# pranshu-raj-211/dmdqn

Measured on NVIDIA B200. Metric: agent-updates/sec, higher is better.
Workload: dtype f32

## Files before the change

dmdqn_b200/csrc/api.cu:

```cuda
#include <stdarg.h>
#include <string.h>
#include "common.cuh"

namespace dmdqn {

static thread_local char g_error[512] = "";

void set_error(const char* fmt, ...) {
    va_list ap;
    va_start(ap, fmt);
    vsnprintf(g_error, sizeof(g_error), fmt, ap);
    va_end(ap);
}

int validate_dims(const dmdqn_dims* d) {
    DMDQN_CHECK_ARG(d != nullptr, "dims is NULL");
    DMDQN_CHECK_ARG(d->n_agents >= 1, "n_agents=%d must be >= 1", d->n_agents);
    DMDQN_CHECK_ARG(d->n_nets == d->n_agents || d->n_nets == 1,
                    "n_nets=%d must be n_agents (independent) or 1 (shared)", d->n_nets);
    DMDQN_CHECK_ARG(d->obs_dim >= 1 && d->obs_stride >= d->obs_dim && d->obs_stride % 16 == 0 &&
                        d->obs_stride <= 128,
                    "obs_dim=%d obs_stride=%d: stride must be a multiple of 16 in [obs_dim, 128]",
                    d->obs_dim, d->obs_stride);
    DMDQN_CHECK_ARG(d->hidden == 64 || d->hidden == 128 || d->hidden == 256 || d->hidden == 512,
// ... 132 lines not shown

static int check_learn_args(const dmdqn_dims* dims, const dmdqn_hparams* hp, const dmdqn_replay* replay,
                            const dmdqn_nets* nets, const void* draws) {
    DMDQN_CHECK_ARG(hp && replay && nets && draws, "NULL argument");
    if (int rc = check_n_step(hp)) return rc;
    DMDQN_CHECK_ARG(replay->obs && replay->next_obs && replay->act && replay->rew && replay->done &&
                        replay->n_written, "NULL replay pointer");
    DMDQN_CHECK_ARG(nets->theta && nets->theta_tgt && nets->adam_m && nets->adam_v && nets->learn_step,
                    "NULL network pointer");
    DMDQN_CHECK_ARG(hp->sample_mode >= 0 && hp->sample_mode <= DMDQN_SAMPLE_PRIORITIZED, "sample_mode=%d", hp->sample_mode);
    if (hp->sample_mode == DMDQN_SAMPLE_PRIORITIZED) {
        DMDQN_CHECK_ARG(replay->priority && replay->priority_max,
                        "sample_mode=prioritized needs the replay's priority and priority_max arrays (NULL priority pointer)");
        DMDQN_CHECK_ARG(!(dims->n_nets == 1 && dims->n_agents > 1),
                        "sample_mode=prioritized serves independent networks only (n_nets=%d, n_agents=%d share parameters)",
                        dims->n_nets, dims->n_agents);
    }
    DMDQN_CHECK_ARG(hp->loss == DMDQN_LOSS_MSE || hp->loss == DMDQN_LOSS_HUBER, "loss=%d", hp->loss);
    DMDQN_CHECK_ARG(hp->precision >= DMDQN_PRECISION_FP32 && hp->precision <= DMDQN_PRECISION_TF32X3, "precision=%d",
                    hp->precision);
    return DMDQN_OK;
}

static int run_learn(const dmdqn_dims* dims, const dmdqn_hparams* hp, const dmdqn_replay* replay, const dmdqn_nets* nets,
                     const void* draws, const uint8_t* learn_mask, float* metrics_out, void* workspace,
                     size_t workspace_bytes, int32_t stages, float* grads, int32_t global_batch, void* stream) {
    Workspace w;
    int rc = check_workspace(dims, workspace, workspace_bytes, &w);
    if (rc) return rc;
    rc = check_learn_args(dims, hp, replay, nets, draws);
    if (rc) return rc;
    if (grads) DMDQN_CHECK_ARG(global_batch >= dims->batch, "global_batch=%d < batch=%d", global_batch, dims->batch);
    if (stages & DMDQN_STAGE_SAMPLE) {
        rc = launch_sample(*dims, *hp, *replay, *nets, draws, learn_mask, 1, (char*)workspace, w, (cudaStream_t)stream);
        if (rc) return rc;
    }
    return launch_learn(*dims, *hp, *replay, *nets, metrics_out, (char*)workspace, w, stages, grads, global_batch,
                        (cudaStream_t)stream);
}

int dmdqn_sample(const dmdqn_dims* dims, const dmdqn_hparams* hp, const dmdqn_replay* replay,
                 const dmdqn_nets* nets, const void* draws, const uint8_t* learn_mask, int32_t advance_step,
                 void* workspace, size_t workspace_bytes, void* stream) {
    Workspace w;
    int rc = check_workspace(dims, workspace, workspace_bytes, &w);
    if (rc) return rc;
    rc = check_learn_args(dims, hp, replay, nets, draws);
    if (rc) return rc;
    return launch_sample(*dims, *hp, *replay, *nets, draws, learn_mask, advance_step, (char*)workspace, w,
                         (cudaStream_t)stream);
}

int dmdqn_gather(const dmdqn_dims* dims, const dmdqn_replay* replay, const void* workspace,
                 size_t workspace_bytes, float* states, int32_t* actions, float* rewards, float* next_states,
                 float* dones, int32_t* active_out, void* stream) {
    Workspace w;
    int rc = check_workspace(dims, const_cast<void*>(workspace), workspace_bytes, &w);
    if (rc) return rc;
    DMDQN_CHECK_ARG(replay && replay->obs && replay->next_obs, "gather: NULL replay pointer");
    DMDQN_CHECK_ARG(states && actions && rewards && next_states && dones, "gather: NULL output");
    return launch_gather(*dims, *replay, (const char*)workspace, w, states, actions, rewards, next_states, dones,
                         active_out, (cudaStream_t)stream);
}

int dmdqn_learn_stages(const dmdqn_dims* dims, const dmdqn_hparams* hp, const dmdqn_replay* replay,
                       const dmdqn_nets* nets, const void* draws, const uint8_t* learn_mask, float* metrics_out,
                       void* workspace, size_t workspace_bytes, int32_t stages, void* stream) {
    return run_learn(dims, hp, replay, nets, draws, learn_mask, metrics_out, workspace, workspace_bytes, stages, nullptr, 0,
                     stream);
}

int dmdqn_learn(const dmdqn_dims* dims, const dmdqn_hparams* hp, const dmdqn_replay* replay,
                const dmdqn_nets* nets, const void* draws, const uint8_t* learn_mask, float* metrics_out,
                void* workspace, size_t workspace_bytes, void* stream) {
    return run_learn(dims, hp, replay, nets, draws, learn_mask, metrics_out, workspace, workspace_bytes, kAllStages, nullptr,
                     0, stream);
}

int dmdqn_step_host(const dmdqn_dims* dims, const dmdqn_hparams* hp, const dmdqn_replay* replay,
                    const dmdqn_nets* nets, const dmdqn_step_block* blk, const void* host_block, void* device_block,
                    float* metrics_dev, float* metrics_host, void* workspace, size_t workspace_bytes, void* stream) {
    int rc = validate_dims(dims);
// ... 140 lines not shown
```

dmdqn_b200/csrc/common.cuh:

```cuda
#pragma once
#include <cuda_runtime.h>
#include <stdint.h>
#include <stdio.h>
#include "../../include/dmdqn_b200.h"

namespace dmdqn {

void set_error(const char* fmt, ...);

#define DMDQN_CHECK_ARG(cond, ...)                                  \
    do {                                                            \
        if (!(cond)) {                                              \
            ::dmdqn::set_error(__VA_ARGS__);                        \
            return DMDQN_ERR_ARG;                                   \
        }                                                           \
    } while (0)

#define DMDQN_CUDA(expr)                                                              \
    do {                                                                              \
        cudaError_t _e = (expr);                                                      \
        if (_e != cudaSuccess) {                                                      \
            ::dmdqn::set_error("%s failed: %s", #expr, cudaGetErrorString(_e));       \
            return DMDQN_ERR_CUDA;                                                    \
        }                                                                             \
// ... 46 lines not shown
    int tiles;
};
inline int tile_bm(int h) { return h >= 512 ? 32 : 64; }
inline Workspace make_workspace(const dmdqn_dims& d) {
    Workspace w;
    size_t off = 0;
    auto take = [&](size_t bytes) { size_t o = off; off += (bytes + 255) / 256 * 256; return o; };
    const size_t nb = (size_t)d.n_nets * d.batch;
    w.tiles = row_tiles(d.batch, tile_bm(d.hidden));
    const size_t nt = (size_t)d.n_nets * w.tiles;
    w.rows = take(nb * 4);
    w.r_hat = take(nb * 4);
    w.act_b = take(nb * 4);
    w.done_b = take(nb * 4);
    w.active = take((size_t)d.n_nets * 4);
    w.y = take(nb * 4);
    w.q_all = take(nb * 16);
    w.q_next = take(nb * 16);
    w.tq_all = take(nb * 16);
    w.h1 = take(nb * d.hidden * 4);
    w.tc_error = take(4);
    w.adam_sc = take((size_t)d.n_nets * 16);
    w.mask2 = take(nb * (size_t)(d.hidden / 32) * 4);
    w.ga = take(nb * 8);
    w.w3_copy = take((size_t)d.n_nets * d.hidden * 16);
    w.dh1 = take(nb * d.hidden * 4);
    w.dh2 = take(nb * d.hidden * 4);
    w.part_loss = take(nt * 8 * 4);
    w.part_b3 = take(nt * 4 * 4);
    w.part_w3 = take(nt * d.hidden * 4 * 4);
    w.part_b2 = take(nt * d.hidden * 4);
    w.part_b1 = take(nt * d.hidden * 4);
    w.is_w = take(nb * 4);
    w.sync = take((4 + (size_t)d.n_nets + nt) * 4);
    w.nrows = take(nb * 4);
    w.disc_b = take(nb * 4);
    w.total = off;
    return w;
}

int validate_dims(const dmdqn_dims* d);

constexpr int kAllStages = DMDQN_STAGE_SAMPLE | DMDQN_STAGE_TARGET | DMDQN_STAGE_ONLINE | DMDQN_STAGE_WGRAD;

struct LearnArgs {
    dmdqn_dims d;
    Layout L;
    dmdqn_replay rp;
    dmdqn_nets nets;
    int loss, double_dqn;
    int loss_batch;
    float one_m_b1, one_m_b2, tau;
    int ws_tiles;
    int tc_tiles;
    const int32_t *rows, *nrows, *act_b, *active;
    const float *r_hat, *disc_b;
    const float4* adam_sc;
    float *y, *q_all, *q_next, *tq_all, *h1, *dh1, *dh2;
    float *part_loss, *part_b3, *part_w3, *part_b2, *part_b1;
    uint32_t* mask2;
    float2* ga;
    float* w3_copy;
    int* error;
    float* metrics;
    float* grads;
    int chain;
    int *sched, *k4a_done, *k3_done;
    int per;
    const float* is_w;
    double per_alpha, per_eps;
};
LearnArgs make_learn_args(const dmdqn_dims& d, const dmdqn_hparams& hp, const dmdqn_replay& rp, const dmdqn_nets& nets,
                          char* ws, const Workspace& w, float* metrics, float* grads, int loss_batch);

__device__ __forceinline__ void per_store_priority(const LearnArgs& A, int row, float delta) {
    const float p = (float)pow(fabs((double)delta) + A.per_eps, A.per_alpha);
    if (!isfinite(p)) return;
    A.rp.priority[row] = p;
    atomicMax(reinterpret_cast<int*>(A.rp.priority_max) + row / A.d.capacity, __float_as_int(p));
}

struct AdamStep {
    float alpha, eps, one_m_b1, one_m_b2, tau;
    int sync;
};
__device__ __forceinline__ AdamStep adam_step(const LearnArgs& A, int g) {
    const float4 sc = __ldg(A.adam_sc + g);
    return {sc.x, sc.y, A.one_m_b1, A.one_m_b2, A.tau, __float_as_int(sc.z)};
}

template <typename Load>
__device__ __forceinline__ void finish_metrics(const LearnArgs& A, int g, int tiles, Load ld) {
    double ls = 0, qs = 0, qq = 0, hist[4] = {0, 0, 0, 0};
#pragma unroll 1
    for (int r = 0; r < tiles; ++r) {
        const float* pl = A.part_loss + ((size_t)g * tiles + r) * 8;
        ls += ld(pl); qs += ld(pl + 1); qq += ld(pl + 2);
        for (int a = 0; a < 4; ++a) hist[a] += ld(pl + 3 + a);
    }
    const double cnt = (double)A.d.batch * A.d.n_actions, mean = qs / cnt, var = fmax(qq / cnt - mean * mean, 0.0);
    float* m = A.metrics + g * DMDQN_METRICS_STRIDE;
    m[0] = (float)(ls / A.loss_batch);
    m[1] = (float)mean;
    m[2] = (float)sqrt(var);
    for (int a = 0; a < 4; ++a) m[3 + a] = (float)hist[a];
    m[7] = 1.f;
}

constexpr int kMaxDevices = 64;
int device_sm_count(int* n_sm);
int opt_in_dynamic_smem(const void* kernel, size_t bytes, size_t (&cache)[kMaxDevices]);

int launch_featurize(int32_t n, const int32_t* halting, const int32_t* phase, const double* next_switch,
                     const double* phase_dur, double sim_time, const uint8_t* signal_valid,
                     const int32_t* nbr_idx, const int32_t* phase_lut, const double* snapshot,
                     double lw, double gw, double* own_out, float* obs_out, int32_t obs_out_stride,
                     double* reward_out, double* global_out, int64_t* scratch, cudaStream_t s);
int launch_featurize_alt(int32_t n, const int32_t* halting, const int32_t* phase, const double* next_switch,
                         const uint8_t* signal_valid, double sim_time, const int32_t* nbr_idx, const double* prev_own,
                         double* own_out, float* obs_out, int32_t obs_out_stride, double* reward_out, cudaStream_t s);
int launch_act(const dmdqn_dims& d, const dmdqn_nets& nets, const float* obs, int32_t stride,
               const double* eps, const uint32_t* w1, const uint32_t* w2, int32_t* actions, float* q_out,
               cudaStream_t s);
int launch_push(const dmdqn_dims& d, const dmdqn_replay& rp, const float* obs, const int32_t* act,
                const double* rew, const float* next_obs, const uint8_t* done, int32_t in_stride,
                const uint8_t* mask, cudaStream_t s);
int launch_sample(const dmdqn_dims& d, const dmdqn_hparams& hp, const dmdqn_replay& rp, const dmdqn_nets& nets,
                  const void* draws, const uint8_t* learn_mask, int advance, char* ws, const Workspace& w,
                  cudaStream_t s);
int launch_gather(const dmdqn_dims& d, const dmdqn_replay& rp, const char* ws, const Workspace& w,
                  float* states, int32_t* actions, float* rewards, float* next_states, float* dones,
                  int32_t* active_out, cudaStream_t s);
int launch_learn(const dmdqn_dims& d, const dmdqn_hparams& hp, const dmdqn_replay& rp, const dmdqn_nets& nets,
                 float* metrics, char* ws, const Workspace& w, int stages, float* grads, int loss_batch, cudaStream_t s);
bool tc_supported(const dmdqn_dims& d);
int launch_learn_tc(const LearnArgs& A, int precision, int stages, cudaStream_t s);
int launch_adam_apply(const dmdqn_dims& d, const dmdqn_hparams& hp, const dmdqn_nets& nets, const float* grads, char* ws,
                      const Workspace& w, cudaStream_t s);
int launch_sync_target(const dmdqn_dims& d, const dmdqn_nets& nets, const uint8_t* mask, double tau,
                       cudaStream_t s);
int launch_peer_adam(const dmdqn_dims& d, const dmdqn_hparams& hp, const dmdqn_nets& nets, const dmdqn_peers& peers,
                     const float* my_loss_src, float* loss_out, char* ws, const Workspace& w, cudaStream_t s);

}
```

dmdqn_b200/csrc/learn_tc.cu:

```cuda
#include <cuda.h>
#include <string.h>
#include "common.cuh"

namespace dmdqn {

namespace {

constexpr int H = 256;
constexpr int BM = 128;
constexpr int EW = 16;
constexpr int NT = EW * 32;
constexpr int W_MMA = EW, W_TMA = EW + 1, W_CONV = EW + 2;
constexpr int CONV_WARPS = 6, CONV_GROUP_WARPS = 2;
constexpr int NT_F = (EW + 8) * 32;
constexpr int REGS_EPI = 104, REGS_AUX = 32;
constexpr int KC = 16;
constexpr uint32_t ATOM = BM * 128;
constexpr unsigned long long WAIT_LIMIT_NS = 2000000000ull;

__device__ __forceinline__ uint32_t smem_u32(const void* p) { return (uint32_t)__cvta_generic_to_shared(p); }

__device__ __forceinline__ uint64_t make_desc(uint32_t saddr, uint32_t lbo_bytes, uint32_t sbo_bytes, uint32_t layout) {
    return (uint64_t)((saddr >> 4) & 0x3FFF) | (uint64_t)((lbo_bytes >> 4) & 0x3FFF) << 16 |
           (uint64_t)((sbo_bytes >> 4) & 0x3FFF) << 32 | (uint64_t)1 << 46 | (uint64_t)layout << 61;
// ... 491 lines not shown
__global__ void __launch_bounds__(NT_F, 1) tc_target_kernel(const LearnArgs A, const __grid_constant__ CUtensorMap tm_w1,
                                                            const __grid_constant__ CUtensorMap tm_w2,
                                                            const __grid_constant__ CUtensorMap tm_w1t,
                                                            const __grid_constant__ CUtensorMap tm_w2t) {
    extern __shared__ uint8_t smem_raw[];
    const uint32_t sbase = (smem_u32(smem_raw) + 1023u) & ~1023u;
    const int B = A.d.batch, Dp = A.d.obs_stride;
    const int n_items = 2 * A.d.n_nets * A.tc_tiles;
    const int warp = threadIdx.x >> 5;
    KT_BEGIN;
    const uint32_t tmem = tc_prologue(sbase);
    if (A.chain) {
        asm volatile("griddepcontrol.wait;" ::: "memory");
        pdl_launch_dependents();
    }
    Ring ring;
    bool ok = true;
    if (warp >= EW) {
        regs_dec<REGS_AUX>();
      if (warp == W_MMA) {
        if ((threadIdx.x & 31) == 0) {
            int prev = -1;
            for (int q = k3_next(A, blockIdx.x, n_items); q < n_items; q = k3_next(A, q + gridDim.x, n_items)) {
                ok = mma_gemm<PASSES, false>(sbase, tmem, sbase + Fwd::R, sbase + Fwd::XLO, 0, Dp, ring, ok);
                if (prev >= 0) flag_release_add(A.k3_done + (size_t)((prev >> 1) / A.tc_tiles) * A.ws_tiles + (prev >> 1) % A.tc_tiles);
                prev = q;
                ok = mma_gemm<PASSES, false>(sbase, tmem, sbase + Fwd::R, 0, tmem + 256u, H, ring, ok);
            }
            if (!ok) atomicExch(A.error, 13);
        }
        __syncwarp();
      } else if (warp == W_TMA) {
        if ((threadIdx.x & 31) == 0) {
            for (int q = k3_next(A, blockIdx.x, n_items); q < n_items;) {
                const int g = (q >> 1) / A.tc_tiles;
                const float* P = ((q & 1) ? A.nets.theta_tgt : A.nets.theta) + (size_t)g * A.L.stride;
                const int qn = k3_next(A, q + gridDim.x, n_items);
                const float* Pn = qn < n_items ? ((qn & 1) ? A.nets.theta_tgt : A.nets.theta) + (size_t)((qn >> 1) / A.tc_tiles) * A.L.stride + A.L.w1 : nullptr;
                ok = tma_fwd(sbase, (q & 1) ? &tm_w1t : &tm_w1, g, P + A.L.w1, Dp, ring, ok, P + A.L.w2);
                ok = tma_fwd(sbase, (q & 1) ? &tm_w2t : &tm_w2, g, P + A.L.w2, H, ring, ok, Pn);
                q = qn;
            }
            if (!ok) atomicExch(A.error, 23);
        }
        __syncwarp();
      } else if (warp < W_CONV + CONV_WARPS) {
        const int tc = threadIdx.x - W_CONV * 32, cg = (warp - W_CONV) / CONV_GROUP_WARPS, t = tc % (CONV_GROUP_WARPS * 32);
        for (int q = k3_next(A, blockIdx.x, n_items); q < n_items; q = k3_next(A, q + gridDim.x, n_items)) {
            ok = conv_ring<PASSES>(sbase, cg, t, ring, ok, Dp / 8);
            ok = conv_ring<PASSES>(sbase, cg, t, ring, ok, H / 8);
        }
        if (!ok && tc == 0) atomicExch(A.error, 33);
      }
    } else {
        regs_inc<REGS_EPI>();
        const Epi e;
        XGather<PASSES> xg;
        int q = k3_next(A, blockIdx.x, n_items);
        if (q < n_items) {
            const int g = (q >> 1) / A.tc_tiles, rt = (q >> 1) % A.tc_tiles;
            xg.begin(A.rp.next_obs, A.nrows + (size_t)g * B, rt * BM, B, Dp, ((q & 1) ? A.nets.theta_tgt : A.nets.theta) + (size_t)g * A.L.stride, A.L);
        }
        int q_last = -1;
        while (q < n_items) {
            const int item = q >> 1, pass = q & 1;
            const int g = item / A.tc_tiles, rt = item % A.tc_tiles, r0 = rt * BM;
// ... 388 lines not shown
    q = __shfl_sync(0xffffffffu, q, 0);
    if (q < 0) ok = __shfl_sync(0xffffffffu, (int)ok, 0) != 0;
    return q;
}
__device__ __forceinline__ float ldcg_f(const float* p) {
    float v;
    asm volatile("ld.global.cg.f32 %0, [%1];" : "=f"(v) : "l"(p));
    return v;
}

template <int PASSES>
__global__ void __launch_bounds__(Wg::NTW, 1) tc_wgrad_kernel(const LearnArgs A, const __grid_constant__ CUtensorMap tmap_h1,
                                                              const __grid_constant__ CUtensorMap tmap_dh1) {
    extern __shared__ uint8_t smem_raw[];
    const int B = A.d.batch, Dp = A.d.obs_stride, G = A.d.n_nets;
    const int tid = threadIdx.x, warp = tid >> 5, lane = tid & 31;
    const uint32_t sbase = (smem_u32(smem_raw) + 1023u) & ~1023u;
    const uint32_t bars = sbase + Wg::BARS;
    const int n_items = 3 * G;
    const int nchunks = (B + KC - 1) / KC;

    if (tid == 0) {
        for (int s = 0; s < Wg::STAGES; ++s) {
            mbar_init(bars + Wg::FULL + 8 * s, 1);
            mbar_init(bars + Wg::CONV + 8 * s, Wg::CONV_WARPS);
            mbar_init(bars + Wg::EMPTY + 8 * s, 1);
        }
        for (int b = 0; b < 2; ++b) {
            mbar_init(bars + Wg::ACC_FULL + 8 * b, 1);
            mbar_init(bars + Wg::ACC_FREE + 8 * b, Wg::EPI_WARPS);
        }
        for (int b = 0; b < Wg::NQ; ++b) mbar_init(bars + Wg::QFULL + 8 * b, 1);
        asm volatile("fence.mbarrier_init.release.cluster;" ::: "memory");
    }
    if (warp == 0) {
        asm volatile("tcgen05.alloc.cta_group::1.sync.aligned.shared::cta.b32 [%0], %1;" ::"r"(bars + Wg::TMEM), "r"(512));
        asm volatile("tcgen05.relinquish_alloc_permit.cta_group::1.sync.aligned;" ::);
    }
    tc_fence_before();
    __syncthreads();
    tc_fence_after();
    uint32_t tmem;
    asm volatile("ld.shared.u32 %0, [%1];" : "=r"(tmem) : "r"(bars + Wg::TMEM));
    bool ok = true;

    if (warp >= Wg::EPI_WARPS + Wg::CONV_WARPS) {
        regs_dec<Wg::REGS_AUX>();
        if (warp == Wg::EPI_WARPS + Wg::CONV_WARPS) {
            {
                uint32_t used = 0;
                int n = 0, nq = 0;
                for (;;) {
                    const int q = wg_pop(bars, nq, ok);
                    if (q < 0) break;
                    if (lane != 0) continue;
                    int g, t;
                    wg_item(q, G, g, t);
                    const bool is_w2 = t < 2;
                    const uint32_t acc_buf = (uint32_t)(n & 1);
                    const uint32_t d_tmem = tmem + acc_buf * 256u;
                    const uint32_t idesc = make_idesc(!is_w2, is_w2);
                    if (n >= 2 && ok)
                        ok = mbar_wait(bars + Wg::ACC_FREE + 8 * acc_buf, (uint32_t)((n >> 1) - 1) & 1u);
                    for (int c = 0; c < nchunks; ++c) {
                        const uint32_t s = used % Wg::STAGES, u = used / Wg::STAGES;
                        if (ok) ok = mbar_wait(bars + Wg::CONV + 8 * s, u & 1u);
                        tc_fence_after();
                        const uint32_t st = sbase + s * Wg::STG;
#pragma unroll
                        for (int ks = 0; ks < 2; ++ks) {
                            uint64_t a_hi, a_lo, b_hi, b_lo;
                            if (is_w2) {
                                a_hi = make_desc(st + ks * 32, 16, 512, 4);
                                a_lo = make_desc(st + Wg::A_BYTES + ks * 32, 16, 512, 4);
// ... 8 lines not shown
                            uint32_t acc = (c | ks) ? 1u : 0u;
                            if (PASSES == 3) {
                                mma_ss(d_tmem, a_lo, b_hi, idesc, acc);
                                mma_ss(d_tmem, a_hi, b_lo, idesc, 1u);
                                acc = 1u;
                            }
                            mma_ss(d_tmem, a_hi, b_hi, idesc, acc);
                        }
                        umma_commit(bars + Wg::EMPTY + 8 * s);
                        if (c == nchunks - 1) umma_commit(bars + Wg::ACC_FULL + 8 * acc_buf);
                        ++used;
                    }
                    ++n;
                }
                if (!ok && lane == 0) atomicExch(A.error, 15);
            }
            __syncwarp();
        } else if (warp == Wg::EPI_WARPS + Wg::CONV_WARPS + 1) {
            uint32_t used = 0;
            int nq = 0;
            int draws = 0;
            for (;;) {
                int q = (int)blockIdx.x + draws * (int)gridDim.x;
                ++draws;
                if (A.chain) {
                    if (lane == 0) q = atomicAdd(A.sched, 1);
                    q = __shfl_sync(0xffffffffu, q, 0);
                }
                if (q >= n_items || !ok) break;
                int g, t;
                wg_item(q, G, g, t);
                if (!A.active[g]) {
                    if (t == 2 && lane < DMDQN_METRICS_STRIDE && A.metrics) A.metrics[g * DMDQN_METRICS_STRIDE + lane] = 0.f;
                    continue;
                }
                if (A.chain) {
                    int fine = 1;
                    if (lane == 0) {
                        fine = flag_acquire_ge(A.k4a_done + g, A.tc_tiles) ? 1 : 0;
                        asm volatile("fence.proxy.async;" ::: "memory");
                    }
                    ok = __shfl_sync(0xffffffffu, fine, 0) != 0;
                    if (!ok) break;
                }
                if (lane == 0) {
                    asm volatile("st.shared.s32 [%0], %1;" ::"r"(bars + Wg::QITEM + 4 * ((uint32_t)nq & (Wg::NQ - 1))), "r"(q) : "memory");
                    mbar_arrive(bars + Wg::QFULL + 8 * ((uint32_t)nq & (Wg::NQ - 1)));
                }
                ++nq;
                const size_t sb = (size_t)g * B;
                int32_t rid = 0;
                if (t == 2 && lane < KC && lane < B) rid = __ldg(A.rows + sb + lane);
                for (int c = 0; c < nchunks; ++c) {
                    const uint32_t s = used % Wg::STAGES, u = used / Wg::STAGES;
                    const uint32_t st = sbase + s * Wg::STG, full = bars + Wg::FULL + 8 * s;
                    const int nvalid = min(KC, B - c * KC);
                    int32_t rid_next = 0;
                    if (t == 2 && c + 1 < nchunks && (c + 1) * KC + lane < B && lane < KC) rid_next = __ldg(A.rows + sb + (c + 1) * KC + lane);
                    if (u && ok) ok = mbar_wait(bars + Wg::EMPTY + 8 * s, (u - 1) & 1u);
                    if (t < 2) {
                        if (lane == 0) {
                            mbar_expect_tx(full, Wg::A_BYTES + (uint32_t)nvalid * 40u);
                            tma_load_3d(st, &tmap_h1, c * KC, t * BM, g, full);
                            bulk_g2s(st + Wg::AUX, A.ga + sb + c * KC, (uint32_t)nvalid * 8u, full);
                            bulk_g2s(st + Wg::AUX + Wg::AUX_MASK, A.mask2 + (sb + c * KC) * 8, (uint32_t)nvalid * 32u, full);
                        }
// ... 210 lines not shown
#pragma unroll
                    for (int u = 0; u < 8; ++u) {
                        const int m = mrow0 + 4 * u;
                        off[u] = wbase + 4 * u * H + c0;
                        if (!is_w2) off[u] = m == Dp ? (int)A.L.b1 + c0 + c4 : (m < Dp ? off[u] : -1);
                        if (is_w2 || off[u] >= 0) {
                            t4[u] = ldg_plain(th + off[u]);
                            m4[u] = ldg_plain(am + off[u]);
                            v4[u] = ldg_plain(av + off[u]);
                        }
                    }
#pragma unroll
                    for (int u = 0; u < 8; ++u) {
                        if (!is_w2 && off[u] < 0) continue;
                        const float4 gr = *reinterpret_cast<const float4*>(trow + 4 * u * Wg::TLD);
                        adam_fast(k, gr.x, t4[u].x, m4[u].x, v4[u].x); adam_fast(k, gr.y, t4[u].y, m4[u].y, v4[u].y);
                        adam_fast(k, gr.z, t4[u].z, m4[u].z, v4[u].z); adam_fast(k, gr.w, t4[u].w, m4[u].w, v4[u].w);
                        *reinterpret_cast<float4*>(th + off[u]) = t4[u];
                        *reinterpret_cast<float4*>(am + off[u]) = m4[u];
                        *reinterpret_cast<float4*>(av + off[u]) = v4[u];
                        if (sync == 1) {
                            *reinterpret_cast<float4*>(tg + off[u]) = t4[u];
                        } else if (sync == 2) {
                            const float omt = 1.0f - k.tau;
                            const float4 g4 = ldg_plain(tg + off[u]);
                            *reinterpret_cast<float4*>(tg + off[u]) =
                                make_float4(k.tau * t4[u].x + omt * g4.x, k.tau * t4[u].y + omt * g4.y,
                                            k.tau * t4[u].z + omt * g4.z, k.tau * t4[u].w + omt * g4.w);
                        }
                    }
                }
                __syncwarp();
            }
            ++n;
        }
        WG_TS();
        WG_TS_PRINT("K4b epilogue (wait, adam)*", et == 0);
#ifdef TC_TIMING
        if (et == 0) { unsigned long long gt; asm volatile("mov.u64 %0, %%globaltimer;" : "=l"(gt));
            printf("K4bsum cta %d sm %d items %d cycles %lld chain %d t0 %llu t1 %llu\n", blockIdx.x, (int)smid_(), n, clock64() - wg_t0, A.chain, wg_g0, gt); }
#endif
        if (!ok && lane == 0) atomicExch(A.error, 6);
    }
    tc_fence_before();
    __syncthreads();
    if (warp == 0) asm volatile("tcgen05.dealloc.cta_group::1.sync.aligned.b32 %0, %1;" ::"r"(tmem), "r"(512));
}

typedef CUresult (*EncodeTiledFn)(CUtensorMap*, CUtensorMapDataType, cuuint32_t, void*, const cuuint64_t*, const cuuint64_t*,
                                  const cuuint32_t*, const cuuint32_t*, CUtensorMapInterleave, CUtensorMapSwizzle,
                                  CUtensorMapL2promotion, CUtensorMapFloatOOBfill);
struct MapKey {
    const void* base;
    cuuint64_t dims[5], strides[4];
    cuuint32_t box[5];
    int rank, swz;
};
int encode_tiled(CUtensorMap* out, const float* base, int rank, const cuuint64_t* dims, const cuuint64_t* strides, const cuuint32_t* box,
                 CUtensorMapSwizzle swz) {
    static EncodeTiledFn encode = nullptr;
    if (!encode) {
        void* fn = nullptr;
        cudaDriverEntryPointQueryResult qres;
        DMDQN_CUDA(cudaGetDriverEntryPoint("cuTensorMapEncodeTiled", &fn, cudaEnableDefault, &qres));
        if (qres != cudaDriverEntryPointSuccess || !fn) {
            set_error("cuTensorMapEncodeTiled is not available from this driver");
            return DMDQN_ERR_CUDA;
        }
        encode = reinterpret_cast<EncodeTiledFn>(fn);
    }
    constexpr int kSlots = 32;
    static thread_local MapKey keys[kSlots];
    static thread_local CUtensorMap maps[kSlots];
    static thread_local int used = 0, next = 0;
    MapKey k = {};
    k.base = base; k.rank = rank; k.swz = (int)swz;
    for (int i = 0; i < rank; ++i) { k.dims[i] = dims[i]; k.box[i] = box[i]; }
    for (int i = 0; i + 1 < rank; ++i) k.strides[i] = strides[i];
    for (int i = 0; i < used; ++i)
// ... 68 lines not shown
        cfg.dynamicSmemBytes = smem_f;
        cfg.numAttrs = A.chain ? 1 : 0;
        CUtensorMap m1, m2;
        if (int rc = make_fwd_tensor_map(A, A.nets.theta, A.L.w1, A.d.obs_stride, &m1)) return rc;
        if (int rc = make_fwd_tensor_map(A, A.nets.theta, A.L.w2, H, &m2)) return rc;
        DMDQN_CUDA(cudaLaunchKernelEx(&cfg, tc_online_kernel<PASSES>, A, tmap, m1, m2));
    }
    if (stages & DMDQN_STAGE_WGRAD) {
        const int items = A.d.n_nets * 3;
        CUtensorMap tmap_h1, tmap_dh1;
        if (int rc = make_scratch_tensor_map(A, A.h1, BM, &tmap_h1)) return rc;
        if (int rc = make_scratch_tensor_map(A, A.dh1, H, &tmap_dh1)) return rc;
        cfg.gridDim = dim3(items < n_sm ? items : n_sm);
        cfg.blockDim = dim3(Wg::NTW);
        cfg.dynamicSmemBytes = smem_w;
        cfg.numAttrs = A.chain ? 1 : 0;
        DMDQN_CUDA(cudaLaunchKernelEx(&cfg, tc_wgrad_kernel<PASSES>, A, tmap_h1, tmap_dh1));
    }
    return DMDQN_OK;
}

}

bool tc_supported(const dmdqn_dims& d) {
    return d.hidden == H && d.obs_stride % 32 == 0 && d.obs_stride <= 96 && d.batch % 4 == 0 && d.batch <= 4096;
}

int launch_learn_tc(const LearnArgs& args, int precision, int stages, cudaStream_t s) {
    LearnArgs A = args;
    A.tc_tiles = (A.d.batch + BM - 1) / BM;
    A.chain = (stages & kAllStages) == kAllStages ? 1 : 0;
    A.k4a_done = A.sched + 4;
    A.k3_done = A.k4a_done + A.d.n_nets;
    return precision == DMDQN_PRECISION_TF32 ? launch_tc<1>(A, stages, s) : launch_tc<3>(A, stages, s);
}

}
```

dmdqn_b200/csrc/replay.cu:

```cuda
#include "common.cuh"

namespace dmdqn {

namespace {

__global__ void __launch_bounds__(64)
push_kernel(dmdqn_dims d, dmdqn_replay rp, const float* __restrict__ obs, const int32_t* __restrict__ act,
            const double* __restrict__ rew, const float* __restrict__ next_obs,
            const uint8_t* __restrict__ done, int in_stride, const uint8_t* __restrict__ mask) {
    const int a = blockIdx.x;
    if (mask && !mask[a]) return;
    const long long nw = rp.n_written[a];
    const size_t row = (size_t)a * d.capacity + (size_t)(nw % d.capacity);
    float* dst_s = rp.obs + row * d.obs_stride;
    float* dst_n = rp.next_obs + row * d.obs_stride;
    for (int c = threadIdx.x; c < d.obs_stride; c += blockDim.x) {
        const bool in = c < d.obs_dim;
        dst_s[c] = in ? obs[(size_t)a * in_stride + c] : 0.f;
        dst_n[c] = in ? next_obs[(size_t)a * in_stride + c] : 0.f;
    }
    __syncthreads();
    if (threadIdx.x == 0) {
        rp.act[row] = act[a];
        rp.rew[row] = rew[a];
// ... 12 lines not shown
    double acc = 0.0;
    for (int i = lane; i < n; i += 32) acc = __dadd_rn(acc, elem(i));
    for (int off = 16; off; off >>= 1) acc = __dadd_rn(acc, __shfl_xor_sync(0xffffffffu, acc, off));
    return acc;
}

__device__ __forceinline__ double nstep_return(const dmdqn_dims& d, const dmdqn_hparams& hp, const dmdqn_replay& rp, int row,
                                               int m, double z0, double mean, double denom, bool normalize) {
    if (m <= 1) return z0;
    const int C = d.capacity, agent = row / C, slot = row - agent * C;
    const double* rw = rp.rew + (size_t)agent * C;
    double r[DMDQN_MAX_NSTEP - 1];
#pragma unroll
    for (int k = 1; k < DMDQN_MAX_NSTEP; ++k) r[k - 1] = k < m ? rw[slot + k < C ? slot + k : slot + k - C] : 0.0;
    double ret = z0, gk = 1.0;
#pragma unroll
    for (int k = 1; k < DMDQN_MAX_NSTEP; ++k) {
        if (k < m) {
            gk = __dmul_rn(gk, hp.gamma);
            const double z = normalize ? __ddiv_rn(__dsub_rn(r[k - 1], mean), denom) : r[k - 1];
            ret = __dadd_rn(ret, __dmul_rn(gk, z));
        }
    }
    return ret;
}

template <bool PER, bool NSTEP>
__global__ void __launch_bounds__(kSampleThreads)
sample_kernel(dmdqn_dims d, dmdqn_hparams hp, dmdqn_replay rp, int32_t* __restrict__ learn_step,
              const uint32_t* __restrict__ draws, const uint8_t* __restrict__ learn_mask, int advance,
              int32_t* __restrict__ rows, float* __restrict__ r_hat, int32_t* __restrict__ act_b,
              float* __restrict__ done_b, int32_t* __restrict__ active, float4* __restrict__ adam_sc,
              int32_t* __restrict__ sync, int tiles, float* __restrict__ is_w, int32_t* __restrict__ nrows,
              float* __restrict__ disc_b) {
    extern __shared__ __align__(16) unsigned char smem_raw[];
    const int B = d.batch, Bp = (B + 1) & ~1;
    int* js = reinterpret_cast<int*>(smem_raw);
    int* pt = js + Bp;
    int* words = pt + Bp;
    double* rs = reinterpret_cast<double*>(words + Bp);
    __shared__ double stat[2];
    __shared__ int per_last, per_pmin;
    __shared__ double per_beta;
    const int g = blockIdx.x, tid = threadIdx.x, lane = tid & 31;
    const bool per = hp.sample_mode == DMDQN_SAMPLE_PRIORITIZED;
    const bool shared_net = d.n_nets == 1 && d.n_agents > 1;
    asm volatile("griddepcontrol.launch_dependents;" ::: "memory");
    if (tid < 4 && g == 0) sync[tid] = 0;
    if (tid == 4) sync[4 + g] = 0;
    if (tid >= 32 && tid < 32 + tiles) sync[4 + d.n_nets + g * tiles + (tid - 32)] = 0;

    const long long nw0 = rp.n_written[shared_net ? 0 : g];
    const int size0 = (int)(nw0 < d.capacity ? nw0 : d.capacity);
    const long long pop = shared_net ? (long long)size0 * d.n_agents : size0;
    const bool on = (learn_mask == nullptr || learn_mask[g]) && pop >= B;
    int t_step = 0;
    if (tid == 0) {
        active[g] = on ? 1 : 0;
        int t = learn_step[g];
        if (on && advance) learn_step[g] = ++t;
        t_step = t;
    }
    if (!on) return;
    auto adam_scalars = [&]() {
        const int t = t_step;
        const double bc1 = 1.0 - pow(hp.beta1, (double)t), bc2 = 1.0 - pow(hp.beta2, (double)t);
        const int freq = hp.target_update_frequency > 0 ? hp.target_update_frequency : 1;
        const int sync_mode = hp.tau >= 0.0 ? 2 : (t % freq == 0 ? 1 : 0);
        adam_sc[g] = make_float4((float)(hp.learning_rate * sqrt(bc2) / bc1),
                                 (float)(hp.adam_form == DMDQN_ADAM_KERAS ? hp.adam_eps : hp.adam_eps * sqrt(bc2)),
                                 __int_as_float(sync_mode), 0.f);
    };

    if constexpr (PER) {
        const int C = d.capacity, nch = (C + kPerChunk - 1) / kPerChunk, warp = tid >> 5;
        const float* __restrict__ pr = rp.priority + (size_t)g * C;
        double* prefix = rs + Bp;
        if (tid == 0) { per_last = -1; per_pmin = 0x7f800000; }
        int last = -1;
        for (int c0 = warp * kPerScan; c0 < nch; c0 += (kSampleThreads / 32) * kPerScan) {
            float v[kPerScan][4];
#pragma unroll
            for (int u = 0; u < kPerScan; ++u)
#pragma unroll
                for (int k = 0; k < 4; ++k) {
                    const int sl = (c0 + u) * kPerChunk + 32 * k + lane;
                    v[u][k] = sl < C ? __ldg(pr + sl) : 0.f;
                }
#pragma unroll
            for (int u = 0; u < kPerScan; ++u) {
                double acc = 0.0;
#pragma unroll
                for (int k = 0; k < 4; ++k) {
                    acc = __dadd_rn(acc, (double)v[u][k]);
                    if (v[u][k] > 0.f) last = (c0 + u) * kPerChunk + 32 * k + lane;
                }
                for (int off = 16; off; off >>= 1) acc = __dadd_rn(acc, __shfl_xor_sync(0xffffffffu, acc, off));
                if (lane == 0 && c0 + u < nch) prefix[c0 + u + 1] = acc;
            }
        }
        last = __reduce_max_sync(0xffffffffu, last);
        __syncthreads();
        if (lane == 0 && last >= 0) atomicMax(&per_last, last);
        if (tid == 32) {
// ... 59 lines not shown
            if (i < B) { pt[i] = ptk; words[i] = pj; }
        }
        if (tid == 0) adam_scalars();
        __syncthreads();
        for (int i = tid; i < B; i += kSampleThreads) {
            int k = words[i];
            int v = js[i];
            if (k >= 0) {
                while (pt[k] >= 0) k = pt[k];
                v = n - k - 1;
            }
            words[i] = v;
        }
    } else if (hp.sample_mode == DMDQN_SAMPLE_REPLACEMENT) {
        for (int i = tid; i < B; i += kSampleThreads) words[i] = (int)__umulhi(draws[(size_t)g * B + i], (unsigned)pop);
        if (tid == 0) adam_scalars();
    } else {
        for (int i = tid; i < B; i += kSampleThreads) {
            const int v = (int)draws[(size_t)g * B + i];
            words[i] = v < 0 ? 0 : (v >= pop ? (int)pop - 1 : v);
        }
        if (tid == 0) adam_scalars();
    }
    __syncthreads();

    for (int i = tid; i < B; i += kSampleThreads) {
        const int logical = words[i];
        const int agent = shared_net ? logical / size0 : g;
        const int lj = shared_net ? logical % size0 : logical;
        const long long nw = shared_net ? rp.n_written[agent] : nw0;
        const long long sz = nw < d.capacity ? nw : d.capacity;
        const int slot = per ? words[i] : (int)((nw - sz + lj) % d.capacity);
        const int row = agent * d.capacity + slot;
        if constexpr (PER) {
            const float p = rp.priority[row];
            is_w[(size_t)g * B + i] = p > 0.f ? (float)pow(__ddiv_rn((double)__int_as_float(per_pmin), (double)p), per_beta) : 1.f;
        }
        rows[(size_t)g * B + i] = row;
        act_b[(size_t)g * B + i] = rp.act[row];
        if constexpr (!NSTEP) {
            const bool dn = rp.done[row];
            done_b[(size_t)g * B + i] = dn ? 1.f : 0.f;
            js[i] = row;
            pt[i] = dn;
        }
        rs[i] = rp.rew[row];
        if constexpr (NSTEP) {
            const int C = d.capacity;
            const int j = per ? (int)(((long long)slot - (nw - sz) % C + C) % C) : lj;
            const int lim = min(hp.n_step, (int)sz - j);
            const uint8_t* dn = rp.done + (size_t)agent * C;
            unsigned bits = 0;
#pragma unroll
            for (int k = 0; k < DMDQN_MAX_NSTEP; ++k)
                if (k < lim && dn[slot + k < C ? slot + k : slot + k - C]) bits |= 1u << k;
            const int m = bits ? __ffs(bits) : lim;
            double gm = hp.gamma;
            for (int k = 1; k < m; ++k) gm = __dmul_rn(gm, hp.gamma);
            const int last = slot + m - 1;
            nrows[(size_t)g * B + i] = agent * C + (last < C ? last : last - C);
            done_b[(size_t)g * B + i] = bits ? 1.f : 0.f;
            disc_b[(size_t)g * B + i] = bits ? 0.f : (float)gm;
            js[i] = row;
            pt[i] = m;
        }
    }
    __syncthreads();
    if constexpr (!NSTEP) {
        for (int i = tid - 32; tid >= 32 && i < B; i += kSampleThreads - 32) {
            nrows[(size_t)g * B + i] = js[i];
            disc_b[(size_t)g * B + i] = (float)hp.gamma * (1.0f - (pt[i] ? 1.f : 0.f));
        }
    }
    if (hp.normalize_rewards) {
        if (tid < 32) {
            const double mean = __ddiv_rn(tree_sum(B, lane, [&](int i) { return rs[i]; }), (double)B);
            const double var = __ddiv_rn(tree_sum(B, lane, [&](int i) {
                                             const double dv = __dsub_rn(rs[i], mean);
                                             return __dmul_rn(dv, dv);
                                         }), (double)B);
            if (lane == 0) { stat[0] = mean; stat[1] = __dadd_rn(__dsqrt_rn(var), 1e-8); }
        }
        __syncthreads();
        const double mean = stat[0], denom = stat[1];
        for (int i = tid; i < B; i += kSampleThreads) {
            const double z = __ddiv_rn(__dsub_rn(rs[i], mean), denom);
            r_hat[(size_t)g * B + i] = (float)(NSTEP ? nstep_return(d, hp, rp, js[i], pt[i], z, mean, denom, true) : z);
        }
    } else {
        for (int i = tid; i < B; i += kSampleThreads)
            r_hat[(size_t)g * B + i] = (float)(NSTEP ? nstep_return(d, hp, rp, js[i], pt[i], rs[i], 0.0, 1.0, false) : rs[i]);
    }
}

__global__ void __launch_bounds__(128)
gather_kernel(dmdqn_dims d, dmdqn_replay rp, const int32_t* __restrict__ rows, const int32_t* __restrict__ nrows,
              const float* __restrict__ r_hat,
              const int32_t* __restrict__ act_b, const float* __restrict__ done_b,
              const int32_t* __restrict__ active, float* __restrict__ states, int32_t* __restrict__ actions,
              float* __restrict__ rewards, float* __restrict__ next_states, float* __restrict__ dones,
              int32_t* __restrict__ active_out) {
    const int lane = threadIdx.x & 31;
    const long long r = (long long)blockIdx.x * 4 + (threadIdx.x >> 5);
    const long long total = (long long)d.n_nets * d.batch;
    if (r >= total) return;
    const int g = (int)(r / d.batch);
    if (active_out && (r % d.batch) == 0 && lane == 0) active_out[g] = active[g];
    if (!active[g]) return;
    const size_t src = (size_t)rows[r] * d.obs_stride;
    const size_t nsrc = (size_t)nrows[r] * d.obs_stride;
    const int q = d.obs_stride >> 2;
    float4 s4 = make_float4(0.f, 0.f, 0.f, 0.f), n4 = s4;
    if (lane < q) {
        s4 = __ldg(reinterpret_cast<const float4*>(rp.obs + src) + lane);
        n4 = __ldg(reinterpret_cast<const float4*>(rp.next_obs + nsrc) + lane);
    }
#pragma unroll
    for (int k = 0; k < 4; ++k) {
        const int c = 32 * k + lane, from = 8 * k + (lane >> 2);
        const float sx = __shfl_sync(0xffffffffu, s4.x, from), sy = __shfl_sync(0xffffffffu, s4.y, from);
        const float sz = __shfl_sync(0xffffffffu, s4.z, from), sw = __shfl_sync(0xffffffffu, s4.w, from);
        const float nx = __shfl_sync(0xffffffffu, n4.x, from), ny = __shfl_sync(0xffffffffu, n4.y, from);
        const float nz = __shfl_sync(0xffffffffu, n4.z, from), nw = __shfl_sync(0xffffffffu, n4.w, from);
        const int comp = lane & 3;
        if (c < d.obs_dim) {
            states[r * d.obs_dim + c] = comp == 0 ? sx : comp == 1 ? sy : comp == 2 ? sz : sw;
            next_states[r * d.obs_dim + c] = comp == 0 ? nx : comp == 1 ? ny : comp == 2 ? nz : nw;
        }
    }
    if (lane == 0) {
        actions[r] = act_b[r];
        rewards[r] = r_hat[r];
        dones[r] = done_b[r];
    }
}

}

int launch_push(const dmdqn_dims& d, const dmdqn_replay& rp, const float* obs, const int32_t* act,
                const double* rew, const float* next_obs, const uint8_t* done, int32_t in_stride,
                const uint8_t* mask, cudaStream_t s) {
    push_kernel<<<d.n_agents, 64, 0, s>>>(d, rp, obs, act, rew, next_obs, done, in_stride, mask);
    DMDQN_CUDA(cudaGetLastError());
    return DMDQN_OK;
}

int launch_sample(const dmdqn_dims& d, const dmdqn_hparams& hp, const dmdqn_replay& rp, const dmdqn_nets& nets,
                  const void* draws, const uint8_t* learn_mask, int advance, char* ws, const Workspace& w,
                  cudaStream_t s) {
    DMDQN_CHECK_ARG(d.batch <= 4096, "batch %d: the sample kernel serves batches up to 4096", d.batch);
    const bool per = hp.sample_mode == DMDQN_SAMPLE_PRIORITIZED;
    DMDQN_CHECK_ARG(!per || d.capacity <= DMDQN_PER_MAX_CAPACITY,
                    "capacity=%d: prioritized replay serves rings of up to %d slots", d.capacity, DMDQN_PER_MAX_CAPACITY);
    const size_t smem = (size_t)((d.batch + 1) & ~1) * (3 * 4 + 8) +
                        (per ? (size_t)((d.capacity + kPerChunk - 1) / kPerChunk + 1) * 8 : 0);
    const bool nstep = hp.n_step > 1;
    static size_t configured[4][kMaxDevices] = {};
    const auto kernel = per ? (nstep ? sample_kernel<true, true> : sample_kernel<true, false>)
                            : (nstep ? sample_kernel<false, true> : sample_kernel<false, false>);
    if (int rc = opt_in_dynamic_smem(reinterpret_cast<const void*>(kernel), smem, configured[2 * per + nstep])) return rc;
    kernel<<<d.n_nets, kSampleThreads, smem, s>>>(
        d, hp, rp, nets.learn_step, static_cast<const uint32_t*>(draws), learn_mask, advance,
        reinterpret_cast<int32_t*>(ws + w.rows), reinterpret_cast<float*>(ws + w.r_hat),
        reinterpret_cast<int32_t*>(ws + w.act_b), reinterpret_cast<float*>(ws + w.done_b),
        reinterpret_cast<int32_t*>(ws + w.active), reinterpret_cast<float4*>(ws + w.adam_sc),
        reinterpret_cast<int32_t*>(ws + w.sync), w.tiles, reinterpret_cast<float*>(ws + w.is_w),
        reinterpret_cast<int32_t*>(ws + w.nrows), reinterpret_cast<float*>(ws + w.disc_b));
    DMDQN_CUDA(cudaGetLastError());
    return DMDQN_OK;
}

int launch_gather(const dmdqn_dims& d, const dmdqn_replay& rp, const char* ws, const Workspace& w,
                  float* states, int32_t* actions, float* rewards, float* next_states, float* dones,
                  int32_t* active_out, cudaStream_t s) {
    const long long total = (long long)d.n_nets * d.batch;
    gather_kernel<<<(unsigned)((total + 3) / 4), 128, 0, s>>>(
        d, rp, reinterpret_cast<const int32_t*>(ws + w.rows), reinterpret_cast<const int32_t*>(ws + w.nrows),
        reinterpret_cast<const float*>(ws + w.r_hat),
        reinterpret_cast<const int32_t*>(ws + w.act_b), reinterpret_cast<const float*>(ws + w.done_b),
        reinterpret_cast<const int32_t*>(ws + w.active), states, actions, rewards, next_states, dones,
        active_out);
    DMDQN_CUDA(cudaGetLastError());
    return DMDQN_OK;
}

}
```

Measured before the change: 541,600.

## Overlap next step's sample kernel with previous learn via PDL and per-net flags

```diff
diff --git a/dmdqn_b200/csrc/api.cu b/dmdqn_b200/csrc/api.cu
--- a/dmdqn_b200/csrc/api.cu
+++ b/dmdqn_b200/csrc/api.cu
@@ -188,7 +188,8 @@
     if (rc) return rc;
     if (grads) DMDQN_CHECK_ARG(global_batch >= dims->batch, "global_batch=%d < batch=%d", global_batch, dims->batch);
     if (stages & DMDQN_STAGE_SAMPLE) {
-        rc = launch_sample(*dims, *hp, *replay, *nets, draws, learn_mask, 1, (char*)workspace, w, (cudaStream_t)stream);
+        const bool chain = stages == kAllStages && hp->precision != DMDQN_PRECISION_FP32 && tc_supported(*dims);
+        rc = launch_sample(*dims, *hp, *replay, *nets, draws, learn_mask, 1, (char*)workspace, w, chain, (cudaStream_t)stream);
         if (rc) return rc;
     }
     return launch_learn(*dims, *hp, *replay, *nets, metrics_out, (char*)workspace, w, stages, grads, global_batch,
@@ -203,7 +204,7 @@
     if (rc) return rc;
     rc = check_learn_args(dims, hp, replay, nets, draws);
     if (rc) return rc;
-    return launch_sample(*dims, *hp, *replay, *nets, draws, learn_mask, advance_step, (char*)workspace, w,
+    return launch_sample(*dims, *hp, *replay, *nets, draws, learn_mask, advance_step, (char*)workspace, w, false,
                          (cudaStream_t)stream);
 }
 
diff --git a/dmdqn_b200/csrc/common.cuh b/dmdqn_b200/csrc/common.cuh
--- a/dmdqn_b200/csrc/common.cuh
+++ b/dmdqn_b200/csrc/common.cuh
@@ -102,7 +102,7 @@
     w.part_b2 = take(nt * d.hidden * 4);
     w.part_b1 = take(nt * d.hidden * 4);
     w.is_w = take(nb * 4);
-    w.sync = take((4 + (size_t)d.n_nets + nt) * 4);
+    w.sync = take((4 + 2 * (size_t)d.n_nets + nt) * 4);
     w.nrows = take(nb * 4);
     w.disc_b = take(nb * 4);
     w.total = off;
@@ -112,6 +112,8 @@
 int validate_dims(const dmdqn_dims* d);
 
 constexpr int kAllStages = DMDQN_STAGE_SAMPLE | DMDQN_STAGE_TARGET | DMDQN_STAGE_ONLINE | DMDQN_STAGE_WGRAD;
+
+constexpr int kK4bDone = 24;
 
 struct LearnArgs {
     dmdqn_dims d;
@@ -135,7 +137,7 @@
     float* metrics;
     float* grads;
     int chain;
-    int *sched, *k4a_done, *k3_done;
+    int *sched, *k4a_done, *k3_done, *k4b_done;
     int per;
     const float* is_w;
     double per_alpha, per_eps;
@@ -197,7 +199,7 @@
                 const uint8_t* mask, cudaStream_t s);
 int launch_sample(const dmdqn_dims& d, const dmdqn_hparams& hp, const dmdqn_replay& rp, const dmdqn_nets& nets,
                   const void* draws, const uint8_t* learn_mask, int advance, char* ws, const Workspace& w,
-                  cudaStream_t s);
+                  bool chain, cudaStream_t s);
 int launch_gather(const dmdqn_dims& d, const dmdqn_replay& rp, const char* ws, const Workspace& w,
                   float* states, int32_t* actions, float* rewards, float* next_states, float* dones,
                   int32_t* active_out, cudaStream_t s);
diff --git a/dmdqn_b200/csrc/learn_tc.cu b/dmdqn_b200/csrc/learn_tc.cu
--- a/dmdqn_b200/csrc/learn_tc.cu
+++ b/dmdqn_b200/csrc/learn_tc.cu
@@ -547,6 +547,7 @@
         __syncwarp();
       } else if (warp == W_TMA) {
         if ((threadIdx.x & 31) == 0) {
+            if (A.chain) asm volatile("fence.proxy.async;" ::: "memory");
             for (int q = k3_next(A, blockIdx.x, n_items); q < n_items;) {
                 const int g = (q >> 1) / A.tc_tiles;
                 const float* P = ((q & 1) ? A.nets.theta_tgt : A.nets.theta) + (size_t)g * A.L.stride;
@@ -1001,6 +1002,10 @@
         }
         for (int b = 0; b < Wg::NQ; ++b) mbar_init(bars + Wg::QFULL + 8 * b, 1);
         asm volatile("fence.mbarrier_init.release.cluster;" ::: "memory");
+        if (A.chain && blockIdx.x == 0) {
+            atomicExch(A.sched + 2, 1);
+            __threadfence();
+        }
     }
     if (warp == 0) {
         asm volatile("tcgen05.alloc.cta_group::1.sync.aligned.shared::cta.b32 [%0], %1;" ::"r"(bars + Wg::TMEM), "r"(512));
@@ -1009,6 +1014,7 @@
     tc_fence_before();
     __syncthreads();
     tc_fence_after();
+    if (A.chain) pdl_launch_dependents();
     uint32_t tmem;
     asm volatile("ld.shared.u32 %0, [%1];" : "=r"(tmem) : "r"(bars + Wg::TMEM));
     bool ok = true;
@@ -1083,6 +1089,9 @@
                 wg_item(q, G, g, t);
                 if (!A.active[g]) {
                     if (t == 2 && lane < DMDQN_METRICS_STRIDE && A.metrics) A.metrics[g * DMDQN_METRICS_STRIDE + lane] = 0.f;
+                    __syncwarp();
+                    if (A.chain && lane == 0)
+                        asm volatile("red.release.gpu.global.add.s32 [%0], %1;" ::"l"(A.k4b_done + g), "r"(Wg::EPI_WARPS) : "memory");
                     continue;
                 }
                 if (A.chain) {
@@ -1359,6 +1368,7 @@
                 }
                 __syncwarp();
             }
+            if (A.chain && lane == 0) flag_release_add(A.k4b_done + g);
             ++n;
         }
         WG_TS();
@@ -1372,6 +1382,14 @@
     tc_fence_before();
     __syncthreads();
     if (warp == 0) asm volatile("tcgen05.dealloc.cta_group::1.sync.aligned.b32 %0, %1;" ::"r"(tmem), "r"(512));
+    if (A.chain && tid == 0) {
+        __threadfence();
+        if (atomicAdd(A.sched + 3, 1) == (int)gridDim.x - 1) {
+            atomicExch(A.sched + 3, 0);
+            __threadfence();
+            atomicExch(A.sched + 2, 0);
+        }
+    }
 }
 
 typedef CUresult (*EncodeTiledFn)(CUtensorMap*, CUtensorMapDataType, cuuint32_t, void*, const cuuint64_t*, const cuuint64_t*,
@@ -1506,6 +1524,8 @@
     A.chain = (stages & kAllStages) == kAllStages ? 1 : 0;
     A.k4a_done = A.sched + 4;
     A.k3_done = A.k4a_done + A.d.n_nets;
+    A.k4b_done = A.k3_done + (size_t)A.d.n_nets * A.ws_tiles;
+    static_assert(3 * Wg::EPI_WARPS == kK4bDone, "k4b_done counts one release per K4b epilogue warp and item");
     return precision == DMDQN_PRECISION_TF32 ? launch_tc<1>(A, stages, s) : launch_tc<3>(A, stages, s);
 }
 
diff --git a/dmdqn_b200/csrc/replay.cu b/dmdqn_b200/csrc/replay.cu
--- a/dmdqn_b200/csrc/replay.cu
+++ b/dmdqn_b200/csrc/replay.cu
@@ -68,13 +68,16 @@
               int32_t* __restrict__ rows, float* __restrict__ r_hat, int32_t* __restrict__ act_b,
               float* __restrict__ done_b, int32_t* __restrict__ active, float4* __restrict__ adam_sc,
               int32_t* __restrict__ sync, int tiles, float* __restrict__ is_w, int32_t* __restrict__ nrows,
-              float* __restrict__ disc_b) {
+              float* __restrict__ disc_b, int* __restrict__ error) {
     extern __shared__ __align__(16) unsigned char smem_raw[];
     const int B = d.batch, Bp = (B + 1) & ~1;
     int* js = reinterpret_cast<int*>(smem_raw);
     int* pt = js + Bp;
     int* words = pt + Bp;
-    double* rs = reinterpret_cast<double*>(words + Bp);
+    int* nr = words + Bp;
+    float* dn = reinterpret_cast<float*>(nr + Bp);
+    float* dc = dn + Bp;
+    double* rs = reinterpret_cast<double*>(dc + Bp);
     __shared__ double stat[2];
     __shared__ int per_last, per_pmin;
     __shared__ double per_beta;
@@ -82,9 +85,36 @@
     const bool per = hp.sample_mode == DMDQN_SAMPLE_PRIORITIZED;
     const bool shared_net = d.n_nets == 1 && d.n_agents > 1;
     asm volatile("griddepcontrol.launch_dependents;" ::: "memory");
-    if (tid < 4 && g == 0) sync[tid] = 0;
-    if (tid == 4) sync[4 + g] = 0;
-    if (tid >= 32 && tid < 32 + tiles) sync[4 + d.n_nets + g * tiles + (tid - 32)] = 0;
+    __shared__ int chain_open;
+    if (tid == 0) {
+        int v;
+        asm volatile("ld.acquire.gpu.global.s32 %0, [%1];" : "=r"(v) : "l"(sync + 2) : "memory");
+        chain_open = v;
+    }
+    __syncthreads();
+    const bool open = !PER && chain_open != 0;
+    if (!open) asm volatile("griddepcontrol.wait;" ::: "memory");
+    int32_t* k4b_done = sync + 4 + d.n_nets + d.n_nets * tiles;
+    if (!open) {
+        if (tid < 2 && g == 0) sync[tid] = 0;
+        if (tid == 4) sync[4 + g] = 0;
+        if (tid == 5) k4b_done[g] = 0;
+        if (tid >= 32 && tid < 32 + tiles) sync[4 + d.n_nets + g * tiles + (tid - 32)] = 0;
+    }
+    auto prev_step_done = [&]() {
+        bool fine = false;
+        for (int i = 0; i < (1 << 21) && !fine; ++i) {
+            int v, c;
+            asm volatile("ld.acquire.gpu.global.s32 %0, [%1];" : "=r"(v) : "l"(k4b_done + g) : "memory");
+            asm volatile("ld.acquire.gpu.global.s32 %0, [%1];" : "=r"(c) : "l"(sync + 2) : "memory");
+            fine = v >= kK4bDone && (g != (int)gridDim.x - 1 || c == 0);
+            if (!fine) __nanosleep(256);
+        }
+        if (!fine) atomicExch(error, 7);
+        k4b_done[g] = 0;
+        sync[4 + g] = 0;
+        for (int r = 0; r < tiles; ++r) sync[4 + d.n_nets + g * tiles + r] = 0;
+    };
 
     const long long nw0 = rp.n_written[shared_net ? 0 : g];
     const int size0 = (int)(nw0 < d.capacity ? nw0 : d.capacity);
@@ -92,20 +122,27 @@
     const bool on = (learn_mask == nullptr || learn_mask[g]) && pop >= B;
     int t_step = 0;
     if (tid == 0) {
-        active[g] = on ? 1 : 0;
         int t = learn_step[g];
         if (on && advance) learn_step[g] = ++t;
         t_step = t;
     }
-    if (!on) return;
+    if (!on) {
+        if (tid == 0) {
+            if (open) prev_step_done();
+            active[g] = 0;
+        }
+        return;
+    }
+    float4 sc = make_float4(0.f, 0.f, 0.f, 0.f);
     auto adam_scalars = [&]() {
         const int t = t_step;
         const double bc1 = 1.0 - pow(hp.beta1, (double)t), bc2 = 1.0 - pow(hp.beta2, (double)t);
         const int freq = hp.target_update_frequency > 0 ? hp.target_update_frequency : 1;
         const int sync_mode = hp.tau >= 0.0 ? 2 : (t % freq == 0 ? 1 : 0);
-        adam_sc[g] = make_float4((float)(hp.learning_rate * sqrt(bc2) / bc1),
-                                 (float)(hp.adam_form == DMDQN_ADAM_KERAS ? hp.adam_eps : hp.adam_eps * sqrt(bc2)),
-                                 __int_as_float(sync_mode), 0.f);
+        sc = make_float4((float)(hp.learning_rate * sqrt(bc2) / bc1),
+                         (float)(hp.adam_form == DMDQN_ADAM_KERAS ? hp.adam_eps : hp.adam_eps * sqrt(bc2)),
+                         __int_as_float(sync_mode), 0.f);
+        if (PER) adam_sc[g] = sc;
     };
 
     if constexpr (PER) {
@@ -231,46 +268,35 @@
         const long long sz = nw < d.capacity ? nw : d.capacity;
         const int slot = per ? words[i] : (int)((nw - sz + lj) % d.capacity);
         const int row = agent * d.capacity + slot;
-        if constexpr (PER) {
-            const float p = rp.priority[row];
-            is_w[(size_t)g * B + i] = p > 0.f ? (float)pow(__ddiv_rn((double)__int_as_float(per_pmin), (double)p), per_beta) : 1.f;
-        }
-        rows[(size_t)g * B + i] = row;
-        act_b[(size_t)g * B + i] = rp.act[row];
+        words[i] = rp.act[row];
+        js[i] = row;
         if constexpr (!NSTEP) {
-            const bool dn = rp.done[row];
-            done_b[(size_t)g * B + i] = dn ? 1.f : 0.f;
-            js[i] = row;
-            pt[i] = dn;
+            const bool d1 = rp.done[row];
+            dn[i] = d1 ? 1.f : 0.f;
+            nr[i] = row;
+            dc[i] = (float)hp.gamma * (1.0f - (d1 ? 1.f : 0.f));
         }
         rs[i] = rp.rew[row];
         if constexpr (NSTEP) {
             const int C = d.capacity;
             const int j = per ? (int)(((long long)slot - (nw - sz) % C + C) % C) : lj;
             const int lim = min(hp.n_step, (int)sz - j);
-            const uint8_t* dn = rp.done + (size_t)agent * C;
+            const uint8_t* dring = rp.done + (size_t)agent * C;
             unsigned bits = 0;
 #pragma unroll
             for (int k = 0; k < DMDQN_MAX_NSTEP; ++k)
-                if (k < lim && dn[slot + k < C ? slot + k : slot + k - C]) bits |= 1u << k;
+                if (k < lim && dring[slot + k < C ? slot + k : slot + k - C]) bits |= 1u << k;
             const int m = bits ? __ffs(bits) : lim;
             double gm = hp.gamma;
             for (int k = 1; k < m; ++k) gm = __dmul_rn(gm, hp.gamma);
             const int last = slot + m - 1;
-            nrows[(size_t)g * B + i] = agent * C + (last < C ? last : last - C);
-            done_b[(size_t)g * B + i] = bits ? 1.f : 0.f;
-            disc_b[(size_t)g * B + i] = bits ? 0.f : (float)gm;
-            js[i] = row;
+            nr[i] = agent * C + (last < C ? last : last - C);
+            dn[i] = bits ? 1.f : 0.f;
+            dc[i] = bits ? 0.f : (float)gm;
             pt[i] = m;
         }
     }
     __syncthreads();
-    if constexpr (!NSTEP) {
-        for (int i = tid - 32; tid >= 32 && i < B; i += kSampleThreads - 32) {
-            nrows[(size_t)g * B + i] = js[i];
-            disc_b[(size_t)g * B + i] = (float)hp.gamma * (1.0f - (pt[i] ? 1.f : 0.f));
-        }
-    }
     if (hp.normalize_rewards) {
         if (tid < 32) {
             const double mean = __ddiv_rn(tree_sum(B, lane, [&](int i) { return rs[i]; }), (double)B);
@@ -284,11 +310,30 @@
         const double mean = stat[0], denom = stat[1];
         for (int i = tid; i < B; i += kSampleThreads) {
             const double z = __ddiv_rn(__dsub_rn(rs[i], mean), denom);
-            r_hat[(size_t)g * B + i] = (float)(NSTEP ? nstep_return(d, hp, rp, js[i], pt[i], z, mean, denom, true) : z);
+            rs[i] = (float)(NSTEP ? nstep_return(d, hp, rp, js[i], pt[i], z, mean, denom, true) : z);
         }
     } else {
         for (int i = tid; i < B; i += kSampleThreads)
-            r_hat[(size_t)g * B + i] = (float)(NSTEP ? nstep_return(d, hp, rp, js[i], pt[i], rs[i], 0.0, 1.0, false) : rs[i]);
+            rs[i] = (float)(NSTEP ? nstep_return(d, hp, rp, js[i], pt[i], rs[i], 0.0, 1.0, false) : rs[i]);
+    }
+    if (tid == 0) {
+        if (open) prev_step_done();
+        active[g] = 1;
+        if (!PER) adam_sc[g] = sc;
+    }
+    __syncthreads();
+    for (int i = tid; i < B; i += kSampleThreads) {
+        const size_t o = (size_t)g * B + i;
+        rows[o] = js[i];
+        act_b[o] = words[i];
+        done_b[o] = dn[i];
+        nrows[o] = nr[i];
+        disc_b[o] = dc[i];
+        r_hat[o] = (float)rs[i];
+        if constexpr (PER) {
+            const float p = rp.priority[js[i]];
+            is_w[o] = p > 0.f ? (float)pow(__ddiv_rn((double)__int_as_float(per_pmin), (double)p), per_beta) : 1.f;
+        }
     }
 }
 
@@ -346,26 +391,36 @@
 
 int launch_sample(const dmdqn_dims& d, const dmdqn_hparams& hp, const dmdqn_replay& rp, const dmdqn_nets& nets,
                   const void* draws, const uint8_t* learn_mask, int advance, char* ws, const Workspace& w,
-                  cudaStream_t s) {
+                  bool chain, cudaStream_t s) {
     DMDQN_CHECK_ARG(d.batch <= 4096, "batch %d: the sample kernel serves batches up to 4096", d.batch);
     const bool per = hp.sample_mode == DMDQN_SAMPLE_PRIORITIZED;
     DMDQN_CHECK_ARG(!per || d.capacity <= DMDQN_PER_MAX_CAPACITY,
                     "capacity=%d: prioritized replay serves rings of up to %d slots", d.capacity, DMDQN_PER_MAX_CAPACITY);
-    const size_t smem = (size_t)((d.batch + 1) & ~1) * (3 * 4 + 8) +
+    const size_t smem = (size_t)((d.batch + 1) & ~1) * (6 * 4 + 8) +
                         (per ? (size_t)((d.capacity + kPerChunk - 1) / kPerChunk + 1) * 8 : 0);
     const bool nstep = hp.n_step > 1;
     static size_t configured[4][kMaxDevices] = {};
     const auto kernel = per ? (nstep ? sample_kernel<true, true> : sample_kernel<true, false>)
                             : (nstep ? sample_kernel<false, true> : sample_kernel<false, false>);
     if (int rc = opt_in_dynamic_smem(reinterpret_cast<const void*>(kernel), smem, configured[2 * per + nstep])) return rc;
-    kernel<<<d.n_nets, kSampleThreads, smem, s>>>(
-        d, hp, rp, nets.learn_step, static_cast<const uint32_t*>(draws), learn_mask, advance,
+    cudaLaunchAttribute pdl[1];
+    pdl[0].id = cudaLaunchAttributeProgrammaticStreamSerialization;
+    pdl[0].val.programmaticStreamSerializationAllowed = 1;
+    cudaLaunchConfig_t cfg = {};
+    cfg.gridDim = dim3(d.n_nets);
+    cfg.blockDim = dim3(kSampleThreads);
+    cfg.dynamicSmemBytes = smem;
+    cfg.stream = s;
+    cfg.attrs = pdl;
+    cfg.numAttrs = chain ? 1 : 0;
+    DMDQN_CUDA(cudaLaunchKernelEx(
+        &cfg, kernel, d, hp, rp, nets.learn_step, static_cast<const uint32_t*>(draws), learn_mask, advance,
         reinterpret_cast<int32_t*>(ws + w.rows), reinterpret_cast<float*>(ws + w.r_hat),
         reinterpret_cast<int32_t*>(ws + w.act_b), reinterpret_cast<float*>(ws + w.done_b),
         reinterpret_cast<int32_t*>(ws + w.active), reinterpret_cast<float4*>(ws + w.adam_sc),
         reinterpret_cast<int32_t*>(ws + w.sync), w.tiles, reinterpret_cast<float*>(ws + w.is_w),
-        reinterpret_cast<int32_t*>(ws + w.nrows), reinterpret_cast<float*>(ws + w.disc_b));
-    DMDQN_CUDA(cudaGetLastError());
+        reinterpret_cast<int32_t*>(ws + w.nrows), reinterpret_cast<float*>(ws + w.disc_b),
+        reinterpret_cast<int*>(ws + w.tc_error)));
     return DMDQN_OK;
 }
 
```

After: 554,700 (median of 6 runs). 1.02x the previous value.
